# pjyazdian/Gesture2Vec

Measured on AMD Instinct MI355X. Metric: gesture-chunks/sec VQ-VAE fwd+bwd (T=34,D=135,K=512), higher is better.
Workload: dtype f32; 1 GPU; BASELINE configs[1] (VQ-VAE full shape): train_iter_Autoencoder_VQ_seq2seq on synthetic N(0,1) pose chunks, B=4096/GPU, T=34, D=135, H=64, L=2 (E=128), K=512, dropout_prob=0 (+ always-on Dropout(0.95)), Adam lr=0.0005, random-init weights; global_batch=4096, per_gpu_batch=4096, parallelism=single, launch=hipGraph replay, wgrad=f32, graph_branches_mask=15, decoder_rollout=persistent: one launch each way, 1 row tile(s) of 16 per workgroup, dist_world_size=1

## Files before the change

gesture2vec_amd/csrc/dec_persist.hip:

```cpp
#define G2V_PERSIST_DEVICE_CODE
#include "dec_persist.hpp"
#include <utility>
#ifndef G2V_BWD_EPI
#define G2V_BWD_EPI 1
#endif

#ifdef G2V_PSTAMPS
__device__ unsigned long long g2v_pstamps[2 * 4 * 24];
#define PSTAMP(dir, k)                                                                                                   \
  do {                                                                                                                   \
    const int sb_ = blockIdx.x == 0 ? 0 : (blockIdx.x == 5 ? 1 : (blockIdx.x == 128 ? 2 : (blockIdx.x == 255 ? 3 : -1))); \
    if (threadIdx.x == 0 && sb_ >= 0 && t == 10) g2v_pstamps[((dir) * 4 + sb_) * 24 + (k)] = __builtin_amdgcn_s_memtime();  \
  } while (0)
extern "C" int g2v_read_pstamps(unsigned long long* out) {
  return (int)hipMemcpyFromSymbol(out, HIP_SYMBOL(g2v_pstamps), sizeof(unsigned long long) * 2 * 4 * 24);
}
#else
#define PSTAMP(dir, k)
#endif

namespace g2v {

namespace {
constexpr int H = 64, D = 135, Dp = 144, LDH = 68, LDD = 148;
constexpr int KSH = 4, KSD = 9;
constexpr int OUT_TILES = 12;
constexpr int L_XA = 0, L_XH0 = L_XA + 16 * LDH, L_XH1 = L_XH0 + 16 * LDH, L_XX1 = L_XH1 + 16 * LDH;
constexpr int L_XY = L_XX1 + 16 * LDH;
constexpr int L_YT = L_XY + 16 * LDD;
constexpr int L_XT = L_YT + 2176;
constexpr int L_KT = L_XT + 2176;
constexpr int L_POUT = L_KT + 544;
constexpr int L_PPRE = L_POUT + 9 * KSH * 256;
constexpr int L_BIAS = L_PPRE + 4 * KSD * 256;
constexpr int L_ST = L_BIAS + 4 * 192 + 144 + 3 * 64;
constexpr int L_RED = L_ST + 128;
constexpr int L_TOT = L_RED + 16 * 128;
constexpr int L_END = L_TOT + 128;
static_assert(L_END * 4 <= 160 * 1024, "LDS budget of the persistent rollout forward");
constexpr int B_IH0 = 0, B_HH0 = 192, B_IH1 = 384, B_HH1 = 576, B_OUT = 768, B_PRE = 912, B_BNW = 976, B_BNB = 1040;
}

size_t dec_persist_fwd_lds_bytes(int tiles_per_wg) { return (size_t)(L_END + (tiles_per_wg - 1) * 2 * 16 * LDH) * sizeof(float); }

struct DecPersistArgs {
  const float* target;
  const float* h_init;
  g2v_dec_weights w;
  const float* p_pre; const float* p_ih0; const float* p_hh0; const float* p_ih1; const float* p_hh1; const float* p_out;
  g2v_dec_saved sv;
  const uint8_t* keep95;
  const uint8_t* keep_l0;
  PersistX x;
  int T, B, nblk, n_pre, conditioned, training;
  float p_drop;
};

template <int NT, int KS_T>
__device__ __forceinline__ void lds_frag_mma(f32x4 (&acc)[NT], const float* P, int tile0, int tile_stride, const float* Xs,
                                             int ldx, int lane) {
  const float* xrow = Xs + (lane & 15) * ldx + 4 * (lane >> 4);
  float4 wn[NT], xn;
#pragma unroll
  for (int t = 0; t < NT; ++t) wn[t] = *reinterpret_cast<const float4*>(P + ((tile0 + t * tile_stride) * KS_T) * 256 + lane * 4);
  xn = *reinterpret_cast<const float4*>(xrow);
#pragma unroll
  for (int s = 0; s < KS_T; ++s) {
    const float4 xb = xn;
    float4 wv[NT];
#pragma unroll
    for (int t = 0; t < NT; ++t) wv[t] = wn[t];
    if (s + 1 < KS_T) {
#pragma unroll
      for (int t = 0; t < NT; ++t)
        wn[t] = *reinterpret_cast<const float4*>(P + ((tile0 + t * tile_stride) * KS_T + s + 1) * 256 + lane * 4);
      xn = *reinterpret_cast<const float4*>(xrow + 16 * (s + 1));
    }
#pragma unroll
    for (int t = 0; t < NT; ++t) acc[t] = mfma16(wv[t].x, xb.x, acc[t]);
#pragma unroll
    for (int t = 0; t < NT; ++t) acc[t] = mfma16(wv[t].y, xb.y, acc[t]);
#pragma unroll
    for (int t = 0; t < NT; ++t) acc[t] = mfma16(wv[t].z, xb.z, acc[t]);
#pragma unroll
    for (int t = 0; t < NT; ++t) acc[t] = mfma16(wv[t].w, xb.w, acc[t]);
  }
}

template <int NT, int KS_T>
__device__ __forceinline__ void frag_mma_x1st(f32x4 (&acc)[NT], const WFrag<NT, KS_T>& f, const float* Xs, int ldx, int lane) {
  const float* xrow = Xs + (lane & 15) * ldx + 4 * (lane >> 4);
  float4 xb[KS_T];
#pragma unroll
  for (int s = 0; s < KS_T; ++s) xb[s] = *reinterpret_cast<const float4*>(xrow + 16 * s);
#pragma unroll
  for (int s = 0; s < KS_T; ++s) {
#pragma unroll
    for (int t = 0; t < NT; ++t) acc[t] = mfma16(f.w[t][s].x, xb[s].x, acc[t]);
#pragma unroll
    for (int t = 0; t < NT; ++t) acc[t] = mfma16(f.w[t][s].y, xb[s].y, acc[t]);
#pragma unroll
    for (int t = 0; t < NT; ++t) acc[t] = mfma16(f.w[t][s].z, xb[s].z, acc[t]);
#pragma unroll
    for (int t = 0; t < NT; ++t) acc[t] = mfma16(f.w[t][s].w, xb[s].w, acc[t]);
  }
}

template <class F, int... Ks>
__device__ __forceinline__ void static_for_(F&& f, std::integer_sequence<int, Ks...>) {
  (f(std::integral_constant<int, Ks>{}), ...);
}
template <int N, class F>
__device__ __forceinline__ void static_for(F&& f) {
  static_for_(static_cast<F&&>(f), std::make_integer_sequence<int, N>{});
}
template <int KS_T>
__device__ __forceinline__ f32x4 lds_frag_mma_2chain(const float* P, int tile, const float* Xs, int ldx, int lane) {
  const float* xrow = Xs + (lane & 15) * ldx + 4 * (lane >> 4);
  const float* wp = P + (tile * KS_T) * 256 + lane * 4;
  f32x4 a0 = {0.f, 0.f, 0.f, 0.f}, a1 = {0.f, 0.f, 0.f, 0.f};
  float4 w0 = *reinterpret_cast<const float4*>(wp), x0 = *reinterpret_cast<const float4*>(xrow);
  float4 w1 = *reinterpret_cast<const float4*>(wp + 256), x1 = *reinterpret_cast<const float4*>(xrow + 16);
#pragma unroll
  for (int s = 0; s < KS_T; s += 2) {
    const float4 wa = w0, xa = x0, wb = w1, xb = x1;
    const bool two = s + 1 < KS_T;
    if (s + 2 < KS_T) {
      w0 = *reinterpret_cast<const float4*>(wp + (s + 2) * 256);
      x0 = *reinterpret_cast<const float4*>(xrow + 16 * (s + 2));
    }
    if (s + 3 < KS_T) {
      w1 = *reinterpret_cast<const float4*>(wp + (s + 3) * 256);
      x1 = *reinterpret_cast<const float4*>(xrow + 16 * (s + 3));
    }
    a0 = mfma16(wa.x, xa.x, a0);
    if (two) a1 = mfma16(wb.x, xb.x, a1);
    a0 = mfma16(wa.y, xa.y, a0);
    if (two) a1 = mfma16(wb.y, xb.y, a1);
    a0 = mfma16(wa.z, xa.z, a0);
    if (two) a1 = mfma16(wb.z, xb.z, a1);
    a0 = mfma16(wa.w, xa.w, a0);
    if (two) a1 = mfma16(wb.w, xb.w, a1);
  }
  return (f32x4){a0[0] + a1[0], a0[1] + a1[1], a0[2] + a1[2], a0[3] + a1[3]};
}

__device__ __forceinline__ void cell_epilogue(const f32x4 (&ai)[3], const f32x4 (&ah)[3], const float* bias_i,
                                              const float* bias_h, uint32_t kp, bool drop, float keep_scale, float* Xh,
                                              float* Xnext, float* __restrict__ h_out, float* __restrict__ gates,
                                              float* __restrict__ xdrop_out, int i, int f0) {
  const float4 hp4 = *reinterpret_cast<const float4*>(Xh + i * LDH + f0);
  const float hp[4] = {hp4.x, hp4.y, hp4.z, hp4.w};
  float4 bi[3], bh[3];
#pragma unroll
  for (int g = 0; g < 3; ++g) {
    bi[g] = *reinterpret_cast<const float4*>(bias_i + g * H + f0);
    bh[g] = *reinterpret_cast<const float4*>(bias_h + g * H + f0);
  }
  const float bir[4] = {bi[0].x, bi[0].y, bi[0].z, bi[0].w}, biz[4] = {bi[1].x, bi[1].y, bi[1].z, bi[1].w},
              bin[4] = {bi[2].x, bi[2].y, bi[2].z, bi[2].w};
  const float bhr[4] = {bh[0].x, bh[0].y, bh[0].z, bh[0].w}, bhz[4] = {bh[1].x, bh[1].y, bh[1].z, bh[1].w},
              bhn[4] = {bh[2].x, bh[2].y, bh[2].z, bh[2].w};
  float hn[4], xd[4], gr_[4], gz_[4], gn_[4], gh_[4];
#pragma unroll
  for (int r = 0; r < 4; ++r) {
    const float rr = sigmoidf_((ai[0][r] + bir[r]) + (ah[0][r] + bhr[r]));
    const float zz = sigmoidf_((ai[1][r] + biz[r]) + (ah[1][r] + bhz[r]));
    const float ghn = ah[2][r] + bhn[r];
    const float nn = tanhf_((ai[2][r] + bin[r]) + rr * ghn);
    hn[r] = (1.0f - zz) * nn + zz * hp[r];
    xd[r] = drop ? (((kp >> (8 * r)) & 0xffu) ? hn[r] * keep_scale : 0.f) : hn[r];
    gr_[r] = rr; gz_[r] = zz; gn_[r] = nn; gh_[r] = ghn;
  }
  *reinterpret_cast<float4*>(Xh + i * LDH + f0) = make_float4(hn[0], hn[1], hn[2], hn[3]);
  if (Xnext) *reinterpret_cast<float4*>(Xnext + i * LDH + f0) = make_float4(xd[0], xd[1], xd[2], xd[3]);
  if (h_out) *reinterpret_cast<float4*>(h_out + (int64_t)i * H + f0) = make_float4(hn[0], hn[1], hn[2], hn[3]);
  if (xdrop_out) *reinterpret_cast<float4*>(xdrop_out + (int64_t)i * H + f0) = make_float4(xd[0], xd[1], xd[2], xd[3]);
  if (gates) {
    float* go = gates + (int64_t)i * 4 * H + f0;
    *reinterpret_cast<float4*>(go) = make_float4(gr_[0], gr_[1], gr_[2], gr_[3]);
    *reinterpret_cast<float4*>(go + H) = make_float4(gz_[0], gz_[1], gz_[2], gz_[3]);
    *reinterpret_cast<float4*>(go + 2 * H) = make_float4(gn_[0], gn_[1], gn_[2], gn_[3]);
    *reinterpret_cast<float4*>(go + 3 * H) = make_float4(gh_[0], gh_[1], gh_[2], gh_[3]);
  }
}

__device__ __forceinline__ void ldg_sync5(const float* p0, const float* p1, const float* p2, const float* p3, const float* p4,
                                          float (&v)[4], uint32_t& w) {
  asm volatile(
      "global_load_dword %0, %5, off\n\tglobal_load_dword %1, %6, off\n\tglobal_load_dword %2, %7, off\n\t"
      "global_load_dword %3, %8, off\n\tglobal_load_dword %4, %9, off\n\ts_waitcnt vmcnt(0)"
      : "=&v"(v[0]), "=&v"(v[1]), "=&v"(v[2]), "=&v"(v[3]), "=&v"(w)
      : "v"(p0), "v"(p1), "v"(p2), "v"(p3), "v"(p4)
      : "memory");
}

__global__ __launch_bounds__(256, 1) void dec_persist_fwd_kernel(DecPersistArgs a) {
  extern __shared__ __attribute__((aligned(16))) float smem[];
  float* Xa = smem + L_XA;
  float* Xh0 = smem + L_XH0;
  float* Xh1 = smem + L_XH1;
  float* Xx1 = smem + L_XX1;
  float* Xy = smem + L_XY;
  float* Xt = smem + L_XT;
  uint32_t* Kt = reinterpret_cast<uint32_t*>(smem + L_KT);
  float* Pout = smem + L_POUT;
  float* Ppre = smem + L_PPRE;
  float* Bs = smem + L_BIAS;
  float* st = smem + L_ST;
  float* red = smem + L_RED;
  float* tot = smem + L_TOT;

  const int tid = threadIdx.x, lane = tid & 63, wave = tid >> 6;
  const int i = lane & 15, q = lane >> 4;
  const int b = blockIdx.x, b0 = b * 16;
  const int T = a.T, B = a.B;
  const int f0 = 16 * wave + 4 * q;
  const bool training = a.training != 0;
  const bool chase = training && a.sv.loss_code != nullptr;
  unsigned* const yflag = a.x.yflag + (size_t)b * PX_FLAG_STRIDE;
  const bool drop = training && a.keep_l0 && a.p_drop > 0.f;
  const float keep_scale = 1.0f / (1.0f - a.p_drop);
  const int64_t BH = (int64_t)B * H;
  const float unbias = (B > 1) ? (float)B / (float)(B - 1) : 1.0f;
  float run_m = 0.f, run_v = 0.f;
  if (training && b == 0 && tid < H && a.w.bn_running_mean) {
    run_m = a.w.bn_running_mean[tid];
    run_v = a.w.bn_running_var[tid];
  }

  WFrag<3, KSH> f_ih0, f_hh0, f_ih1, f_hh1;
  frag_load(f_hh0, a.p_hh0, wave, 4, lane);
  frag_load(f_hh1, a.p_hh1, wave, 4, lane);
  frag_load(f_ih0, a.p_ih0, wave, 4, lane);
  frag_load(f_ih1, a.p_ih1, wave, 4, lane);
  for (int e = tid; e < 9 * KSH * 64; e += 256)
    reinterpret_cast<float4*>(Pout)[e] = reinterpret_cast<const float4*>(a.p_out)[e];
  for (int e = tid; e < 4 * KSD * 64; e += 256) reinterpret_cast<float4*>(Ppre)[e] = reinterpret_cast<const float4*>(a.p_pre)[e];
  for (int e = tid; e < 192; e += 256) {
    Bs[B_IH0 + e] = a.w.b_ih0[e]; Bs[B_HH0 + e] = a.w.b_hh0[e];
    Bs[B_IH1 + e] = a.w.b_ih1[e]; Bs[B_HH1 + e] = a.w.b_hh1[e];
  }
  for (int e = tid; e < 144; e += 256) Bs[B_OUT + e] = e < D ? a.w.b_out[e] : 0.f;
  if (tid < H) {
    Bs[B_PRE + tid] = a.w.b_pre[tid];
    Bs[B_BNW + tid] = a.w.bn_w[tid];
    Bs[B_BNB + tid] = a.w.bn_b[tid];
    if (!training) {
      st[tid] = a.w.bn_running_mean[tid];
      st[H + tid] = bn_invstd_(a.w.bn_running_var[tid]);
    }
  }
  for (int e = tid; e < 16 * (LDD - D); e += 256) Xy[(e / (LDD - D)) * LDD + D + (e % (LDD - D))] = 0.f;
  for (int e = tid; e < 4 * 16 * LDH; e += 256) smem[L_XA + e] = 0.f;
  lds_barrier();
  {
    const int r = tid >> 4, c = (tid & 15) * 4;
    const float4 v0 = *reinterpret_cast<const float4*>(a.h_init + (int64_t)(b0 + r) * H + c);
    const float4 v1 = *reinterpret_cast<const float4*>(a.h_init + BH + (int64_t)(b0 + r) * H + c);
    *reinterpret_cast<float4*>(Xh0 + r * LDH + c) = v0;
    *reinterpret_cast<float4*>(Xh1 + r * LDH + c) = v1;
    if (a.sv.h0) *reinterpret_cast<float4*>(a.sv.h0 + (int64_t)(b0 + r) * H + c) = v0;
    if (a.sv.h1) *reinterpret_cast<float4*>(a.sv.h1 + (int64_t)(b0 + r) * H + c) = v1;
  }

  f32x4 u_acc = {0.f, 0.f, 0.f, 0.f};
  bool pend_dense = false;
  auto dense_stores = [&](int ts, bool nxt) {
    const int64_t tile = ((int64_t)ts * B + b0) * D;
    const float* Ys = smem + L_YT;
    for (int e4 = tid; e4 < (16 * D) / 4; e4 += 256) {
      st4(a.sv.y + tile + 4 * e4, reinterpret_cast<const float4*>(Ys)[e4], chase);
      if (nxt && a.sv.xin) *reinterpret_cast<float4*>(a.sv.xin + tile + 4 * e4) = reinterpret_cast<const float4*>(Xt)[e4];
    }
  };

  for (int t = 0; t < T; ++t) {
    const bool has_next = t < T - 1;
    float* Yt = smem + L_YT;
    if (t > 0) {
      PSTAMP(0, 0);
      f32x4 gh0[3], gh1[3];
#pragma unroll
      for (int g = 0; g < 3; ++g) {
        gh0[g] = (f32x4){0.f, 0.f, 0.f, 0.f};
        gh1[g] = (f32x4){0.f, 0.f, 0.f, 0.f};
      }
      uint32_t kreq[3] = {0u, 0u, 0u};
      const bool fast_y = has_next && !(t < a.n_pre);
      if (fast_y && a.conditioned) {
        const uint32_t* kp4 = reinterpret_cast<const uint32_t*>(a.keep95 + ((int64_t)t * B + b0) * D);
#pragma unroll
        for (int j = 0; j < 3; ++j) {
          const int e4 = tid + 256 * j;
          kreq[j] = kp4[e4 < (16 * D) / 4 ? e4 : 0];
        }
      }
      frag_mma_x1st(gh0, f_hh0, Xh0, LDH, lane);
      PSTAMP(0, 9);
      if (training) {
        if (chase) asm volatile("s_waitcnt vmcnt(0)" ::: "memory");
        px_hop1(a.x, t & 1, (unsigned)t, a.nblk, b, red, tot, tid);
      }
      PSTAMP(0, 10);
      frag_mma_x1st(gh1, f_hh1, Xh1, LDH, lane);
      PSTAMP(0, 1);
#pragma unroll
      for (int j = 0; j < 3; ++j) {
        const int e4 = tid + 256 * j;
        if (e4 < (16 * D) / 4) Kt[e4] = kreq[j];
      }
      __builtin_amdgcn_s_waitcnt(0x0F70);
      if (training) {
        if (px_two_hops(a.nblk)) px_hop2(a.x, t & 1, (unsigned)t, a.nblk, b, red, tot, tid);
        PSTAMP(0, 11);
        if (tid < H) {
          const float s1 = tot[tid], s2 = tot[H + tid];
          const float mv = s1 / (float)B;
          const float var = fmaxf(s2 / (float)B - mv * mv, 0.f);
          const float mean = mv + Bs[B_PRE + tid];
          st[tid] = mean;
          st[H + tid] = bn_invstd_(var);
          if (b == 0 && a.sv.bn_stats) {
            a.sv.bn_stats[(int64_t)(t - 1) * 2 * H + tid] = mean;
            a.sv.bn_stats[(int64_t)(t - 1) * 2 * H + H + tid] = var;
          }
          run_m = 0.9f * run_m + 0.1f * mean;
          run_v = 0.9f * run_v + 0.1f * (var * unbias);
        }
        lds_barrier();
        if (chase && t >= 2 && tid == 0) __hip_atomic_store(yflag, (unsigned)(t - 2), __ATOMIC_RELAXED, __HIP_MEMORY_SCOPE_AGENT);
      }
      if (pend_dense) {
        dense_stores(t - 1, true);
        pend_dense = false;
      }
      PSTAMP(0, 2);
      {
        const float4 m4 = *reinterpret_cast<const float4*>(st + f0), i4 = *reinterpret_cast<const float4*>(st + H + f0);
        const float4 g4 = *reinterpret_cast<const float4*>(Bs + B_BNW + f0), b4 = *reinterpret_cast<const float4*>(Bs + B_BNB + f0);
        const float4 p4 = *reinterpret_cast<const float4*>(Bs + B_PRE + f0);
        float4 a4;
        a4.x = fmaxf(((u_acc[0] + p4.x) - m4.x) * i4.x * g4.x + b4.x, 0.f);
        a4.y = fmaxf(((u_acc[1] + p4.y) - m4.y) * i4.y * g4.y + b4.y, 0.f);
        a4.z = fmaxf(((u_acc[2] + p4.z) - m4.z) * i4.z * g4.z + b4.z, 0.f);
        a4.w = fmaxf(((u_acc[3] + p4.w) - m4.w) * i4.w * g4.w + b4.w, 0.f);
        *reinterpret_cast<float4*>(Xa + i * LDH + f0) = a4;
        if (a.sv.a) *reinterpret_cast<float4*>(a.sv.a + ((int64_t)(t - 1) * B + b0 + i) * H + f0) = a4;
      }
      lds_barrier();
      PSTAMP(0, 3);
      {
        f32x4 ai[3];
#pragma unroll
        for (int g = 0; g < 3; ++g) ai[g] = (f32x4){0.f, 0.f, 0.f, 0.f};
        if (drop) {
          const uint32_t kp = *reinterpret_cast<const uint32_t*>(a.keep_l0 + ((int64_t)(t - 1) * B + b0 + i) * H + f0);
          frag_mma_x1st(ai, f_ih0, Xa, LDH, lane);
          cell_epilogue(ai, gh0, Bs + B_IH0, Bs + B_HH0, kp, true, keep_scale, Xh0, Xx1,
                        a.sv.h0 ? a.sv.h0 + ((int64_t)t * B + b0) * H : nullptr,
                        a.sv.gates0 ? a.sv.gates0 + ((int64_t)(t - 1) * B + b0) * 4 * H : nullptr,
                        a.sv.x1 ? a.sv.x1 + ((int64_t)(t - 1) * B + b0) * H : nullptr, i, f0);
        } else {
          frag_mma_x1st(ai, f_ih0, Xa, LDH, lane);
          cell_epilogue(ai, gh0, Bs + B_IH0, Bs + B_HH0, 0x01010101u, false, 1.0f, Xh0, Xx1,
                        a.sv.h0 ? a.sv.h0 + ((int64_t)t * B + b0) * H : nullptr,
                        a.sv.gates0 ? a.sv.gates0 + ((int64_t)(t - 1) * B + b0) * 4 * H : nullptr, nullptr, i, f0);
        }
      }
      lds_barrier();
      PSTAMP(0, 4);
      {
        f32x4 ai[3];
#pragma unroll
        for (int g = 0; g < 3; ++g) ai[g] = (f32x4){0.f, 0.f, 0.f, 0.f};
        frag_mma_x1st(ai, f_ih1, Xx1, LDH, lane);
        cell_epilogue(ai, gh1, Bs + B_IH1, Bs + B_HH1, 0x01010101u, false, 1.0f, Xh1, nullptr,
                      a.sv.h1 ? a.sv.h1 + ((int64_t)t * B + b0) * H : nullptr,
                      a.sv.gates1 ? a.sv.gates1 + ((int64_t)(t - 1) * B + b0) * 4 * H : nullptr, nullptr, i, f0);
      }
      if (chase && !has_next) asm volatile("s_waitcnt vmcnt(0)" ::: "memory");
      lds_barrier();
      if (chase && !has_next && t >= 2 && tid == 0)
        __hip_atomic_store(yflag, (unsigned)(t - 1), __ATOMIC_RELAXED, __HIP_MEMORY_SCOPE_AGENT);
      PSTAMP(0, 5);
      {
        f32x4 acc[3];
#pragma unroll
        for (int j = 0; j < 3; ++j) acc[j] = (f32x4){0.f, 0.f, 0.f, 0.f};
        if (wave == 0) {
          lds_frag_mma<3, KSH>(acc, Pout, wave, 4, Xh1, LDH, lane);
        } else {
          f32x4 a2[2] = {acc[0], acc[1]};
          lds_frag_mma<2, KSH>(a2, Pout, wave, 4, Xh1, LDH, lane);
          acc[0] = a2[0]; acc[1] = a2[1];
        }
        const uint8_t* Kb = reinterpret_cast<const uint8_t*>(Kt);
        const bool fast_y = has_next && !(t < a.n_pre);
        float bo[3][4], yv[3][4], xv[3][4];
        uint32_t kb[3][4];
#pragma unroll
        for (int j = 0; j < 3; ++j) {
          const int d0 = 16 * (wave + 4 * j) + 4 * q, d0c = d0 < Dp ? d0 : 4 * q;
          const float4 b4 = *reinterpret_cast<const float4*>(Bs + B_OUT + d0c);
          bo[j][0] = b4.x; bo[j][1] = b4.y; bo[j][2] = b4.z; bo[j][3] = b4.w;
#pragma unroll
          for (int r = 0; r < 4; ++r) kb[j][r] = Kb[i * D + d0c + r];
        }
#pragma unroll
        for (int j = 0; j < 3; ++j)
#pragma unroll
          for (int r = 0; r < 4; ++r) {
            yv[j][r] = acc[j][r] + bo[j][r];
            xv[j][r] = kb[j][r] ? yv[j][r] * 20.0f : 0.f;
          }
#pragma unroll
        for (int j = 0; j < 3; ++j) {
          const int d0 = 16 * (wave + 4 * j) + 4 * q;
#pragma unroll
          for (int r = 0; r < 4; ++r)
            if (d0 + r < D) {
              Yt[i * D + d0 + r] = yv[j][r];
              if (fast_y) {
                Xt[i * D + d0 + r] = xv[j][r];
                Xy[i * LDD + d0 + r] = xv[j][r];
              }
            }
        }
      }
      lds_barrier();
      PSTAMP(0, 6);
    }
    const bool fast_dense = t > 0 && (!has_next || !(t < a.n_pre));
    if (fast_dense) {
      if (!has_next) dense_stores(t, false);
    } else {
      const int64_t tile = ((int64_t)t * B + b0) * D;
      const bool teacher = has_next && (t < a.n_pre);
      const uint32_t* kp4 = reinterpret_cast<const uint32_t*>(a.keep95 + tile);
      for (int e4 = tid; e4 < (16 * D) / 4; e4 += 256) {
        const int e = 4 * e4;
        float yv[4], sv_[4], tv[4];
        uint32_t kraw;
        {
          const float* tp[4];
#pragma unroll
          for (int j = 0; j < 4; ++j) {
            const int r = (e + j) / D, c = (e + j) - r * D;
            tp[j] = a.target + ((int64_t)(b0 + r) * T + t) * D + c;
          }
          const bool needk = has_next && a.conditioned;
          ldg_sync5(tp[0], tp[1], tp[2], tp[3], needk ? reinterpret_cast<const float*>(kp4 + e4) : tp[0], tv, kraw);
          if (!needk) kraw = 0u;
        }
        if (t == 0) {
#pragma unroll
          for (int j = 0; j < 4; ++j) yv[j] = tv[j];
        } else {
          const float4 y4 = reinterpret_cast<const float4*>(Yt)[e4];
          yv[0] = y4.x; yv[1] = y4.y; yv[2] = y4.z; yv[3] = y4.w;
        }
        st4(a.sv.y + tile + e, make_float4(yv[0], yv[1], yv[2], yv[3]), chase);
        if (!has_next) continue;
#pragma unroll
        for (int j = 0; j < 4; ++j) {
          sv_[j] = (teacher && t > 0) ? tv[j] : yv[j];
        }
        const uint32_t k4 = kraw;
        float xv[4];
#pragma unroll
        for (int j = 0; j < 4; ++j) xv[j] = ((k4 >> (8 * j)) & 0xffu) ? sv_[j] * 20.0f : 0.f;
        if (a.sv.xin) *reinterpret_cast<float4*>(a.sv.xin + tile + e) = make_float4(xv[0], xv[1], xv[2], xv[3]);
#pragma unroll
        for (int j = 0; j < 4; ++j) {
          const int r = (e + j) / D, c = (e + j) - r * D;
          Xy[r * LDD + c] = xv[j];
        }
      }
    }
    if (!has_next) break;
    if (!fast_dense) lds_barrier();
    PSTAMP(0, 7);
    {
      u_acc = lds_frag_mma_2chain<KSD>(Ppre, wave, Xy, LDD, lane);
      const float4 p4 = *reinterpret_cast<const float4*>(Bs + B_PRE + f0);
      if (a.sv.u)
        *reinterpret_cast<float4*>(a.sv.u + ((int64_t)t * B + b0 + i) * H + f0) =
            make_float4(u_acc[0] + p4.x, u_acc[1] + p4.y, u_acc[2] + p4.z, u_acc[3] + p4.w);
      if (training) {
        float s1[4], s2[4];
#pragma unroll
        for (int r = 0; r < 4; ++r) {
          s1[r] = reduce16(u_acc[r]);
          s2[r] = reduce16(u_acc[r] * u_acc[r]);
        }
        if (i == 0) {
          const int par = (t + 1) & 1;
          __amdgpu_buffer_rsrc_t rr = __builtin_amdgcn_make_buffer_rsrc(
              a.x.rec1 + ((size_t)par * PX_MAX_NBLK + b) * PX_COLS, 0, PX_COLS * 8, 0x00020000);
          const unsigned tag = (unsigned)(t + 1);
          px_publish2(rr, (unsigned)f0, s1[0], s1[1], tag);
          px_publish2(rr, (unsigned)f0 + 2, s1[2], s1[3], tag);
          px_publish2(rr, (unsigned)(H + f0), s2[0], s2[1], tag);
          px_publish2(rr, (unsigned)(H + f0) + 2, s2[2], s2[3], tag);
        }
      }
    }
    if (fast_dense) pend_dense = true;
    PSTAMP(0, 8);
  }
  if (training && b == 0 && tid < H && a.w.bn_running_mean &&
      __hip_atomic_load(&g2v_persist_fault, __ATOMIC_RELAXED, __HIP_MEMORY_SCOPE_AGENT) == 0u) {
    a.w.bn_running_mean[tid] = run_m;
    a.w.bn_running_var[tid] = run_v;
  }
  if (chase) {
    asm volatile("s_waitcnt vmcnt(0)" ::: "memory");
    lds_barrier();
    if (tid == 0) __hip_atomic_store(yflag, (unsigned)(T - 1), __ATOMIC_RELAXED, __HIP_MEMORY_SCOPE_AGENT);
  }
}


template <int R>
__global__ __launch_bounds__(256, 1) void dec_persist_fwd_mt_kernel(DecPersistArgs a, int nwg) {
  extern __shared__ __attribute__((aligned(16))) float smem[];
  float* Xa = smem + L_XA;
  float* Xx1 = smem + L_XX1;
  float* Xy = smem + L_XY;
  float* Xt = smem + L_XT;
  float* Yt = smem + L_YT;
  uint32_t* Kt = reinterpret_cast<uint32_t*>(smem + L_KT);
  float* Pout = smem + L_POUT;
  float* Ppre = smem + L_PPRE;
  float* Bs = smem + L_BIAS;
  float* st = smem + L_ST;
  float* red = smem + L_RED;
  float* tot = smem + L_TOT;
  auto Xh0_of = [&](int r) { return r == 0 ? smem + L_XH0 : smem + L_END + (r - 1) * 2 * 16 * LDH; };
  auto Xh1_of = [&](int r) { return r == 0 ? smem + L_XH1 : smem + L_END + (r - 1) * 2 * 16 * LDH + 16 * LDH; };

  const int tid = threadIdx.x, lane = tid & 63, wave = tid >> 6;
  const int i = lane & 15, q = lane >> 4;
  const int b = blockIdx.x;
  const int T = a.T, B = a.B, ntiles = a.nblk;
  const int f0 = 16 * wave + 4 * q;
  const bool training = a.training != 0;
  const bool drop = training && a.keep_l0 && a.p_drop > 0.f;
  const float keep_scale = 1.0f / (1.0f - a.p_drop);
  const int64_t BH = (int64_t)B * H;
  const float unbias = (B > 1) ? (float)B / (float)(B - 1) : 1.0f;
  float run_m = 0.f, run_v = 0.f;
  if (training && b == 0 && tid < H && a.w.bn_running_mean) {
    run_m = a.w.bn_running_mean[tid];
    run_v = a.w.bn_running_var[tid];
  }
  WFrag<3, KSH> f_ih0, f_hh0, f_ih1, f_hh1;
  frag_load(f_hh0, a.p_hh0, wave, 4, lane);
  frag_load(f_hh1, a.p_hh1, wave, 4, lane);
  frag_load(f_ih0, a.p_ih0, wave, 4, lane);
  frag_load(f_ih1, a.p_ih1, wave, 4, lane);
  for (int e = tid; e < 9 * KSH * 64; e += 256)
    reinterpret_cast<float4*>(Pout)[e] = reinterpret_cast<const float4*>(a.p_out)[e];
  for (int e = tid; e < 4 * KSD * 64; e += 256) reinterpret_cast<float4*>(Ppre)[e] = reinterpret_cast<const float4*>(a.p_pre)[e];
  for (int e = tid; e < 192; e += 256) {
    Bs[B_IH0 + e] = a.w.b_ih0[e]; Bs[B_HH0 + e] = a.w.b_hh0[e];
    Bs[B_IH1 + e] = a.w.b_ih1[e]; Bs[B_HH1 + e] = a.w.b_hh1[e];
  }
  for (int e = tid; e < 144; e += 256) Bs[B_OUT + e] = e < D ? a.w.b_out[e] : 0.f;
  if (tid < H) {
    Bs[B_PRE + tid] = a.w.b_pre[tid];
    Bs[B_BNW + tid] = a.w.bn_w[tid];
    Bs[B_BNB + tid] = a.w.bn_b[tid];
    if (!training) {
      st[tid] = a.w.bn_running_mean[tid];
      st[H + tid] = bn_invstd_(a.w.bn_running_var[tid]);
    }
  }
  for (int e = tid; e < 16 * (LDD - D); e += 256) Xy[(e / (LDD - D)) * LDD + D + (e % (LDD - D))] = 0.f;
  for (int e = tid; e < 4 * 16 * LDH; e += 256) smem[L_XA + e] = 0.f;
  for (int e = tid; e < (R - 1) * 2 * 16 * LDH; e += 256) smem[L_END + e] = 0.f;
  lds_barrier();
  static_for<R>([&](auto rc) {
    constexpr int r = decltype(rc)::value;
    const int tb = b + r * nwg;
    if (tb < ntiles && (tid >> 4) < min(16, B - 16 * tb)) {
      const int rr = tid >> 4, c = (tid & 15) * 4, b0 = 16 * tb;
      const float4 v0 = *reinterpret_cast<const float4*>(a.h_init + (int64_t)(b0 + rr) * H + c);
      const float4 v1 = *reinterpret_cast<const float4*>(a.h_init + BH + (int64_t)(b0 + rr) * H + c);
      *reinterpret_cast<float4*>(Xh0_of(r) + rr * LDH + c) = v0;
      *reinterpret_cast<float4*>(Xh1_of(r) + rr * LDH + c) = v1;
      if (a.sv.h0) *reinterpret_cast<float4*>(a.sv.h0 + (int64_t)(b0 + rr) * H + c) = v0;
      if (a.sv.h1) *reinterpret_cast<float4*>(a.sv.h1 + (int64_t)(b0 + rr) * H + c) = v1;
    }
  });
  lds_barrier();

  f32x4 u_acc[R];
#pragma unroll
  for (int r = 0; r < R; ++r) u_acc[r] = (f32x4){0.f, 0.f, 0.f, 0.f};

  for (int t = 0; t < T; ++t) {
    const bool has_next = t < T - 1;
    float s1a[4] = {0.f, 0.f, 0.f, 0.f}, s2a[4] = {0.f, 0.f, 0.f, 0.f};
    static_for<R>([&](auto rc) {
      constexpr int r = decltype(rc)::value;
      const int tb = b + r * nwg;
      if (tb >= ntiles) return;
      const int b0 = 16 * tb;
      const int nrows = min(16, B - b0);
      const bool rowok = i < nrows;
      const int ic = rowok ? i : nrows - 1;
      const int n4v = (nrows * D) / 4;
      float* Xh0 = Xh0_of(r);
      float* Xh1 = Xh1_of(r);
      if (t > 0) {
        f32x4 gh0[3], gh1[3];
#pragma unroll
        for (int g = 0; g < 3; ++g) {
          gh0[g] = (f32x4){0.f, 0.f, 0.f, 0.f};
          gh1[g] = (f32x4){0.f, 0.f, 0.f, 0.f};
        }
        uint32_t kreq[3] = {0u, 0u, 0u};
        const bool fast_y = has_next && !(t < a.n_pre);
        if (fast_y && a.conditioned) {
          const uint32_t* kp4 = reinterpret_cast<const uint32_t*>(a.keep95 + ((int64_t)t * B + b0) * D);
#pragma unroll
          for (int j = 0; j < 3; ++j) {
            const int e4 = tid + 256 * j;
            kreq[j] = kp4[e4 < n4v ? e4 : 0];
          }
        }
        frag_mma_x1st(gh0, f_hh0, Xh0, LDH, lane);
        if (r == 0 && training) px_hop1(a.x, t & 1, (unsigned)t, nwg, b, red, tot, tid);
        frag_mma_x1st(gh1, f_hh1, Xh1, LDH, lane);
#pragma unroll
        for (int j = 0; j < 3; ++j) {
          const int e4 = tid + 256 * j;
          if (e4 < (16 * D) / 4) Kt[e4] = kreq[j];
        }
        if (r == 0 && training) {
          if (px_two_hops(nwg)) px_hop2(a.x, t & 1, (unsigned)t, nwg, b, red, tot, tid);
          if (tid < H) {
            const float s1 = tot[tid], s2 = tot[H + tid];
            const float mv = s1 / (float)B;
            const float var = fmaxf(s2 / (float)B - mv * mv, 0.f);
            const float mean = mv + Bs[B_PRE + tid];
            st[tid] = mean;
            st[H + tid] = bn_invstd_(var);
            if (b == 0 && a.sv.bn_stats) {
              a.sv.bn_stats[(int64_t)(t - 1) * 2 * H + tid] = mean;
              a.sv.bn_stats[(int64_t)(t - 1) * 2 * H + H + tid] = var;
            }
            run_m = 0.9f * run_m + 0.1f * mean;
            run_v = 0.9f * run_v + 0.1f * (var * unbias);
          }
          lds_barrier();
        }
        {
          const float4 m4 = *reinterpret_cast<const float4*>(st + f0), i4 = *reinterpret_cast<const float4*>(st + H + f0);
          const float4 g4 = *reinterpret_cast<const float4*>(Bs + B_BNW + f0), b4 = *reinterpret_cast<const float4*>(Bs + B_BNB + f0);
          const float4 p4 = *reinterpret_cast<const float4*>(Bs + B_PRE + f0);
          float4 a4;
          a4.x = fmaxf(((u_acc[r][0] + p4.x) - m4.x) * i4.x * g4.x + b4.x, 0.f);
          a4.y = fmaxf(((u_acc[r][1] + p4.y) - m4.y) * i4.y * g4.y + b4.y, 0.f);
          a4.z = fmaxf(((u_acc[r][2] + p4.z) - m4.z) * i4.z * g4.z + b4.z, 0.f);
          a4.w = fmaxf(((u_acc[r][3] + p4.w) - m4.w) * i4.w * g4.w + b4.w, 0.f);
          *reinterpret_cast<float4*>(Xa + i * LDH + f0) = a4;
          if (a.sv.a && rowok) *reinterpret_cast<float4*>(a.sv.a + ((int64_t)(t - 1) * B + b0 + i) * H + f0) = a4;
        }
        lds_barrier();
        {
          f32x4 ai[3];
#pragma unroll
          for (int g = 0; g < 3; ++g) ai[g] = (f32x4){0.f, 0.f, 0.f, 0.f};
          if (drop) {
            const uint32_t kp = *reinterpret_cast<const uint32_t*>(a.keep_l0 + ((int64_t)(t - 1) * B + b0 + ic) * H + f0);
            frag_mma_x1st(ai, f_ih0, Xa, LDH, lane);
            cell_epilogue(ai, gh0, Bs + B_IH0, Bs + B_HH0, kp, true, keep_scale, Xh0, Xx1,
                          (a.sv.h0 && rowok) ? a.sv.h0 + ((int64_t)t * B + b0) * H : nullptr,
                          (a.sv.gates0 && rowok) ? a.sv.gates0 + ((int64_t)(t - 1) * B + b0) * 4 * H : nullptr,
                          (a.sv.x1 && rowok) ? a.sv.x1 + ((int64_t)(t - 1) * B + b0) * H : nullptr, i, f0);
          } else {
            frag_mma_x1st(ai, f_ih0, Xa, LDH, lane);
            cell_epilogue(ai, gh0, Bs + B_IH0, Bs + B_HH0, 0x01010101u, false, 1.0f, Xh0, Xx1,
                          (a.sv.h0 && rowok) ? a.sv.h0 + ((int64_t)t * B + b0) * H : nullptr,
                          (a.sv.gates0 && rowok) ? a.sv.gates0 + ((int64_t)(t - 1) * B + b0) * 4 * H : nullptr, nullptr, i, f0);
          }
        }
        lds_barrier();
        {
          f32x4 ai[3];
#pragma unroll
          for (int g = 0; g < 3; ++g) ai[g] = (f32x4){0.f, 0.f, 0.f, 0.f};
          frag_mma_x1st(ai, f_ih1, Xx1, LDH, lane);
          cell_epilogue(ai, gh1, Bs + B_IH1, Bs + B_HH1, 0x01010101u, false, 1.0f, Xh1, nullptr,
                        (a.sv.h1 && rowok) ? a.sv.h1 + ((int64_t)t * B + b0) * H : nullptr,
                        (a.sv.gates1 && rowok) ? a.sv.gates1 + ((int64_t)(t - 1) * B + b0) * 4 * H : nullptr, nullptr, i, f0);
        }
        lds_barrier();
        {
          f32x4 acc[3];
#pragma unroll
          for (int j = 0; j < 3; ++j) acc[j] = (f32x4){0.f, 0.f, 0.f, 0.f};
          if (wave == 0) {
            lds_frag_mma<3, KSH>(acc, Pout, wave, 4, Xh1, LDH, lane);
          } else {
            f32x4 a2[2] = {acc[0], acc[1]};
            lds_frag_mma<2, KSH>(a2, Pout, wave, 4, Xh1, LDH, lane);
            acc[0] = a2[0]; acc[1] = a2[1];
          }
          const uint8_t* Kb = reinterpret_cast<const uint8_t*>(Kt);
          float bo[3][4], yv[3][4], xv[3][4];
          uint32_t kb[3][4];
#pragma unroll
          for (int j = 0; j < 3; ++j) {
            const int d0 = 16 * (wave + 4 * j) + 4 * q, d0c = d0 < Dp ? d0 : 4 * q;
            const float4 b4 = *reinterpret_cast<const float4*>(Bs + B_OUT + d0c);
            bo[j][0] = b4.x; bo[j][1] = b4.y; bo[j][2] = b4.z; bo[j][3] = b4.w;
#pragma unroll
            for (int e = 0; e < 4; ++e) kb[j][e] = Kb[i * D + d0c + e];
          }
#pragma unroll
          for (int j = 0; j < 3; ++j)
#pragma unroll
            for (int e = 0; e < 4; ++e) {
              yv[j][e] = acc[j][e] + bo[j][e];
              xv[j][e] = kb[j][e] ? yv[j][e] * 20.0f : 0.f;
            }
#pragma unroll
          for (int j = 0; j < 3; ++j) {
            const int d0 = 16 * (wave + 4 * j) + 4 * q;
#pragma unroll
            for (int e = 0; e < 4; ++e)
              if (d0 + e < D) {
                Yt[i * D + d0 + e] = yv[j][e];
                if (fast_y) {
                  Xt[i * D + d0 + e] = xv[j][e];
                  Xy[i * LDD + d0 + e] = xv[j][e];
                }
              }
          }
        }
        lds_barrier();
      }
      const bool fast_dense = t > 0 && (!has_next || !(t < a.n_pre));
      const int64_t tile = ((int64_t)t * B + b0) * D;
      if (fast_dense) {
        for (int e4 = tid; e4 < n4v; e4 += 256) {
          *reinterpret_cast<float4*>(a.sv.y + tile + 4 * e4) = reinterpret_cast<const float4*>(Yt)[e4];
          if (has_next && a.sv.xin) *reinterpret_cast<float4*>(a.sv.xin + tile + 4 * e4) = reinterpret_cast<const float4*>(Xt)[e4];
        }
      } else {
        const bool teacher = has_next && (t < a.n_pre);
        const uint32_t* kp4 = reinterpret_cast<const uint32_t*>(a.keep95 + tile);
        for (int e4 = tid; e4 < n4v; e4 += 256) {
          const int e = 4 * e4;
          float yv[4], sv_[4], tv[4];
          uint32_t kraw;
          {
            const float* tp[4];
#pragma unroll
            for (int j = 0; j < 4; ++j) {
              const int rr = (e + j) / D, c = (e + j) - rr * D;
              tp[j] = a.target + ((int64_t)(b0 + rr) * T + t) * D + c;
            }
            const bool needk = has_next && a.conditioned;
            ldg_sync5(tp[0], tp[1], tp[2], tp[3], needk ? reinterpret_cast<const float*>(kp4 + e4) : tp[0], tv, kraw);
            if (!needk) kraw = 0u;
          }
          if (t == 0) {
#pragma unroll
            for (int j = 0; j < 4; ++j) yv[j] = tv[j];
          } else {
            const float4 y4 = reinterpret_cast<const float4*>(Yt)[e4];
            yv[0] = y4.x; yv[1] = y4.y; yv[2] = y4.z; yv[3] = y4.w;
          }
          *reinterpret_cast<float4*>(a.sv.y + tile + e) = make_float4(yv[0], yv[1], yv[2], yv[3]);
          if (!has_next) continue;
#pragma unroll
          for (int j = 0; j < 4; ++j) {
            sv_[j] = (teacher && t > 0) ? tv[j] : yv[j];
          }
          const uint32_t k4 = kraw;
          float xv[4];
#pragma unroll
          for (int j = 0; j < 4; ++j) xv[j] = ((k4 >> (8 * j)) & 0xffu) ? sv_[j] * 20.0f : 0.f;
// ... 1061 lines not shown
```

Measured before the change: 2.636 million chunks/s.

## Interleave deferred global stores with MFMA chains in persistent decoder forward

Deferred dense y/xin stores and the GRU cell's h/gate/xdrop global stores are no longer issued in bursts after each epilogue. They are now spread between MFMA instructions of the next matrix product, with sched_barrier fences fixing their placement. The aim is to hide store issue and memory latency behind tensor-core work in the serial per-timestep recurrence. In exchange, each cell's outputs stay live in registers across the next GEMM, which raises register pressure and could lower occupancy or cause spills.

```diff
diff --git a/gesture2vec_amd/csrc/dec_persist.hip b/gesture2vec_amd/csrc/dec_persist.hip
--- a/gesture2vec_amd/csrc/dec_persist.hip
+++ b/gesture2vec_amd/csrc/dec_persist.hip
@@ -1,5 +1,6 @@
 #define G2V_PERSIST_DEVICE_CODE
 #include "dec_persist.hpp"
+#include <type_traits>
 #include <utility>
 #ifndef G2V_BWD_EPI
 #define G2V_BWD_EPI 1
@@ -56,9 +57,12 @@
   float p_drop;
 };
 
-template <int NT, int KS_T>
+struct NoIssue {
+  __device__ __forceinline__ void operator()(int) const {}
+};
+template <int NT, int KS_T, class Issue = NoIssue>
 __device__ __forceinline__ void lds_frag_mma(f32x4 (&acc)[NT], const float* P, int tile0, int tile_stride, const float* Xs,
-                                             int ldx, int lane) {
+                                             int ldx, int lane, Issue&& issue = Issue()) {
   const float* xrow = Xs + (lane & 15) * ldx + 4 * (lane >> 4);
   float4 wn[NT], xn;
 #pragma unroll
@@ -84,6 +88,10 @@
     for (int t = 0; t < NT; ++t) acc[t] = mfma16(wv[t].z, xb.z, acc[t]);
 #pragma unroll
     for (int t = 0; t < NT; ++t) acc[t] = mfma16(wv[t].w, xb.w, acc[t]);
+    if constexpr (!std::is_same<std::decay_t<Issue>, NoIssue>::value) {
+      issue(s);
+      __builtin_amdgcn_sched_barrier(0);
+    }
   }
 }
 
@@ -103,6 +111,34 @@
     for (int t = 0; t < NT; ++t) acc[t] = mfma16(f.w[t][s].z, xb[s].z, acc[t]);
 #pragma unroll
     for (int t = 0; t < NT; ++t) acc[t] = mfma16(f.w[t][s].w, xb[s].w, acc[t]);
+  }
+}
+
+template <int NL, int NT, int KS_T, class Issue>
+__device__ __forceinline__ void frag_mma_x1st_issue(f32x4 (&acc)[NT], const WFrag<NT, KS_T>& f, const float* Xs, int ldx, int lane,
+                                                    Issue&& issue) {
+  constexpr int STRIDE = NT * KS_T * 4 / NL;
+  static_assert(STRIDE >= 1, "more stores than MFMAs");
+  const float* xrow = Xs + (lane & 15) * ldx + 4 * (lane >> 4);
+  float4 xb[KS_T];
+#pragma unroll
+  for (int s = 0; s < KS_T; ++s) xb[s] = *reinterpret_cast<const float4*>(xrow + 16 * s);
+  auto after = [&](int m) {
+    if ((m % STRIDE) == STRIDE - 1 && m / STRIDE < NL) {
+      issue(m / STRIDE);
+      __builtin_amdgcn_sched_barrier(0);
+    }
+  };
+#pragma unroll
+  for (int s = 0; s < KS_T; ++s) {
+#pragma unroll
+    for (int t = 0; t < NT; ++t) { acc[t] = mfma16(f.w[t][s].x, xb[s].x, acc[t]); after((s * 4 + 0) * NT + t); }
+#pragma unroll
+    for (int t = 0; t < NT; ++t) { acc[t] = mfma16(f.w[t][s].y, xb[s].y, acc[t]); after((s * 4 + 1) * NT + t); }
+#pragma unroll
+    for (int t = 0; t < NT; ++t) { acc[t] = mfma16(f.w[t][s].z, xb[s].z, acc[t]); after((s * 4 + 2) * NT + t); }
+#pragma unroll
+    for (int t = 0; t < NT; ++t) { acc[t] = mfma16(f.w[t][s].w, xb[s].w, acc[t]); after((s * 4 + 3) * NT + t); }
   }
 }
 
@@ -145,10 +181,26 @@
   return (f32x4){a0[0] + a1[0], a0[1] + a1[1], a0[2] + a1[2], a0[3] + a1[3]};
 }
 
+struct CellSt {
+  float4 h, xd, gr, gz, gn, gh;
+};
+__device__ __forceinline__ void cell_store(const CellSt& c, int k, float* __restrict__ h_out, float* __restrict__ gates,
+                                           float* __restrict__ xdrop_out, int i, int f0) {
+  float* const go = gates + (int64_t)i * 4 * H + f0;
+  switch (k) {
+    case 0: if (h_out) *reinterpret_cast<float4*>(h_out + (int64_t)i * H + f0) = c.h; break;
+    case 1: if (gates) *reinterpret_cast<float4*>(go) = c.gr; break;
+    case 2: if (gates) *reinterpret_cast<float4*>(go + H) = c.gz; break;
+    case 3: if (gates) *reinterpret_cast<float4*>(go + 2 * H) = c.gn; break;
+    case 4: if (gates) *reinterpret_cast<float4*>(go + 3 * H) = c.gh; break;
+    default: if (xdrop_out) *reinterpret_cast<float4*>(xdrop_out + (int64_t)i * H + f0) = c.xd; break;
+  }
+}
+
 __device__ __forceinline__ void cell_epilogue(const f32x4 (&ai)[3], const f32x4 (&ah)[3], const float* bias_i,
                                               const float* bias_h, uint32_t kp, bool drop, float keep_scale, float* Xh,
                                               float* Xnext, float* __restrict__ h_out, float* __restrict__ gates,
-                                              float* __restrict__ xdrop_out, int i, int f0) {
+                                              float* __restrict__ xdrop_out, int i, int f0, CellSt* defer = nullptr) {
   const float4 hp4 = *reinterpret_cast<const float4*>(Xh + i * LDH + f0);
   const float hp[4] = {hp4.x, hp4.y, hp4.z, hp4.w};
   float4 bi[3], bh[3];
@@ -174,6 +226,15 @@
   }
   *reinterpret_cast<float4*>(Xh + i * LDH + f0) = make_float4(hn[0], hn[1], hn[2], hn[3]);
   if (Xnext) *reinterpret_cast<float4*>(Xnext + i * LDH + f0) = make_float4(xd[0], xd[1], xd[2], xd[3]);
+  if (defer) {
+    defer->h = make_float4(hn[0], hn[1], hn[2], hn[3]);
+    defer->xd = make_float4(xd[0], xd[1], xd[2], xd[3]);
+    defer->gr = make_float4(gr_[0], gr_[1], gr_[2], gr_[3]);
+    defer->gz = make_float4(gz_[0], gz_[1], gz_[2], gz_[3]);
+    defer->gn = make_float4(gn_[0], gn_[1], gn_[2], gn_[3]);
+    defer->gh = make_float4(gh_[0], gh_[1], gh_[2], gh_[3]);
+    return;
+  }
   if (h_out) *reinterpret_cast<float4*>(h_out + (int64_t)i * H + f0) = make_float4(hn[0], hn[1], hn[2], hn[3]);
   if (xdrop_out) *reinterpret_cast<float4*>(xdrop_out + (int64_t)i * H + f0) = make_float4(xd[0], xd[1], xd[2], xd[3]);
   if (gates) {
@@ -329,11 +390,8 @@
           run_v = 0.9f * run_v + 0.1f * (var * unbias);
         }
         lds_barrier();
+        PSTAMP(0, 16);
         if (chase && t >= 2 && tid == 0) __hip_atomic_store(yflag, (unsigned)(t - 2), __ATOMIC_RELAXED, __HIP_MEMORY_SCOPE_AGENT);
-      }
-      if (pend_dense) {
-        dense_stores(t - 1, true);
-        pend_dense = false;
       }
       PSTAMP(0, 2);
       {
@@ -350,34 +408,56 @@
       }
       lds_barrier();
       PSTAMP(0, 3);
+      const bool dn = pend_dense;
+      pend_dense = false;
+      const int64_t dtile = ((int64_t)(t - 1) * B + b0) * D;
+      auto dense_read = [&](int k) {
+        const int e4 = tid + 256 * (k >> 1);
+        const float* src = (k & 1) ? Xt : smem + L_YT;
+        return reinterpret_cast<const float4*>(src)[e4 < (16 * D) / 4 ? e4 : tid];
+      };
+      float4 dv = make_float4(0.f, 0.f, 0.f, 0.f);
+      if (dn) dv = dense_read(0);
+      auto dense_issue = [&](int k) {
+        if (!dn) return;
+        const int e4 = tid + 256 * (k >> 1);
+        if (e4 < (16 * D) / 4) {
+          if ((k & 1) == 0) st4(a.sv.y + dtile + 4 * e4, dv, chase);
+          else if (a.sv.xin) *reinterpret_cast<float4*>(a.sv.xin + dtile + 4 * e4) = dv;
+        }
+        if (k + 1 < 6) dv = dense_read(k + 1);
+      };
+      CellSt c0;
+      float* const h0_out = a.sv.h0 ? a.sv.h0 + ((int64_t)t * B + b0) * H : nullptr;
+      float* const g0_out = a.sv.gates0 ? a.sv.gates0 + ((int64_t)(t - 1) * B + b0) * 4 * H : nullptr;
+      float* const x1_out = drop && a.sv.x1 ? a.sv.x1 + ((int64_t)(t - 1) * B + b0) * H : nullptr;
       {
         f32x4 ai[3];
 #pragma unroll
         for (int g = 0; g < 3; ++g) ai[g] = (f32x4){0.f, 0.f, 0.f, 0.f};
         if (drop) {
           const uint32_t kp = *reinterpret_cast<const uint32_t*>(a.keep_l0 + ((int64_t)(t - 1) * B + b0 + i) * H + f0);
-          frag_mma_x1st(ai, f_ih0, Xa, LDH, lane);
-          cell_epilogue(ai, gh0, Bs + B_IH0, Bs + B_HH0, kp, true, keep_scale, Xh0, Xx1,
-                        a.sv.h0 ? a.sv.h0 + ((int64_t)t * B + b0) * H : nullptr,
-                        a.sv.gates0 ? a.sv.gates0 + ((int64_t)(t - 1) * B + b0) * 4 * H : nullptr,
-                        a.sv.x1 ? a.sv.x1 + ((int64_t)(t - 1) * B + b0) * H : nullptr, i, f0);
+          frag_mma_x1st_issue<6>(ai, f_ih0, Xa, LDH, lane, dense_issue);
+          PSTAMP(0, 12);
+          cell_epilogue(ai, gh0, Bs + B_IH0, Bs + B_HH0, kp, true, keep_scale, Xh0, Xx1, h0_out, g0_out, x1_out, i, f0, &c0);
         } else {
-          frag_mma_x1st(ai, f_ih0, Xa, LDH, lane);
-          cell_epilogue(ai, gh0, Bs + B_IH0, Bs + B_HH0, 0x01010101u, false, 1.0f, Xh0, Xx1,
-                        a.sv.h0 ? a.sv.h0 + ((int64_t)t * B + b0) * H : nullptr,
-                        a.sv.gates0 ? a.sv.gates0 + ((int64_t)(t - 1) * B + b0) * 4 * H : nullptr, nullptr, i, f0);
+          frag_mma_x1st_issue<6>(ai, f_ih0, Xa, LDH, lane, dense_issue);
+          PSTAMP(0, 12);
+          cell_epilogue(ai, gh0, Bs + B_IH0, Bs + B_HH0, 0x01010101u, false, 1.0f, Xh0, Xx1, h0_out, g0_out, nullptr, i, f0, &c0);
         }
       }
       lds_barrier();
       PSTAMP(0, 4);
+      CellSt c1;
+      float* const h1_out = a.sv.h1 ? a.sv.h1 + ((int64_t)t * B + b0) * H : nullptr;
+      float* const g1_out = a.sv.gates1 ? a.sv.gates1 + ((int64_t)(t - 1) * B + b0) * 4 * H : nullptr;
       {
         f32x4 ai[3];
 #pragma unroll
         for (int g = 0; g < 3; ++g) ai[g] = (f32x4){0.f, 0.f, 0.f, 0.f};
-        frag_mma_x1st(ai, f_ih1, Xx1, LDH, lane);
-        cell_epilogue(ai, gh1, Bs + B_IH1, Bs + B_HH1, 0x01010101u, false, 1.0f, Xh1, nullptr,
-                      a.sv.h1 ? a.sv.h1 + ((int64_t)t * B + b0) * H : nullptr,
-                      a.sv.gates1 ? a.sv.gates1 + ((int64_t)(t - 1) * B + b0) * 4 * H : nullptr, nullptr, i, f0);
+        frag_mma_x1st_issue<6>(ai, f_ih1, Xx1, LDH, lane, [&](int k) { cell_store(c0, k, h0_out, g0_out, x1_out, i, f0); });
+        PSTAMP(0, 13);
+        cell_epilogue(ai, gh1, Bs + B_IH1, Bs + B_HH1, 0x01010101u, false, 1.0f, Xh1, nullptr, h1_out, g1_out, nullptr, i, f0, &c1);
       }
       if (chase && !has_next) asm volatile("s_waitcnt vmcnt(0)" ::: "memory");
       lds_barrier();
@@ -388,13 +468,18 @@
         f32x4 acc[3];
 #pragma unroll
         for (int j = 0; j < 3; ++j) acc[j] = (f32x4){0.f, 0.f, 0.f, 0.f};
+        auto c1_issue = [&](int s) {
+          if (s == 0) cell_store(c1, 0, h1_out, g1_out, nullptr, i, f0);
+          cell_store(c1, s + 1, h1_out, g1_out, nullptr, i, f0);
+        };
         if (wave == 0) {
-          lds_frag_mma<3, KSH>(acc, Pout, wave, 4, Xh1, LDH, lane);
+          lds_frag_mma<3, KSH>(acc, Pout, wave, 4, Xh1, LDH, lane, c1_issue);
         } else {
           f32x4 a2[2] = {acc[0], acc[1]};
-          lds_frag_mma<2, KSH>(a2, Pout, wave, 4, Xh1, LDH, lane);
+          lds_frag_mma<2, KSH>(a2, Pout, wave, 4, Xh1, LDH, lane, c1_issue);
           acc[0] = a2[0]; acc[1] = a2[1];
         }
+        PSTAMP(0, 14);
         const uint8_t* Kb = reinterpret_cast<const uint8_t*>(Kt);
         const bool fast_y = has_next && !(t < a.n_pre);
         float bo[3][4], yv[3][4], xv[3][4];
@@ -483,6 +568,7 @@
     PSTAMP(0, 7);
     {
       u_acc = lds_frag_mma_2chain<KSD>(Ppre, wave, Xy, LDD, lane);
+      PSTAMP(0, 15);
       const float4 p4 = *reinterpret_cast<const float4*>(Bs + B_PRE + f0);
       if (a.sv.u)
         *reinterpret_cast<float4*>(a.sv.u + ((int64_t)t * B + b0 + i) * H + f0) =
```

Result: faster. 2.674 million chunks/s, median of 6 (+1.4%).
